# cvYouTian/Dedark-YOLO

Hardware: AMD Instinct MI355X
Metric: training img/s at 640x640 (higher is better)
Workload: dtype bf16

## Files before the change

dedark_yolo_amd/_C.py:

```python
import ctypes as C
import os

_HERE = os.path.dirname(os.path.abspath(__file__))
LIB_PATH = os.path.join(os.environ.get("DY_LIB_DIR") or os.path.join(_HERE, "lib"), "libdedark_yolo.so")

DY_F32, DY_BF16, DY_F16 = 0, 1, 2
ACT_NONE, ACT_SILU, ACT_LEAKY = 0, 1, 2
OPT_RULES = dict(Adam=0, Adamax=1, NAdam=2, RAdam=3, RMSProp=4)
STATS_REPLICAS = 64
BN_BWD_REPLICAS = 8

vp, i32, i64, f32, f64 = C.c_void_p, C.c_int, C.c_int64, C.c_float, C.c_double


class ConvDesc(C.Structure):
    _fields_ = [("src", vp), ("src_ld", i64), ("N", i32), ("Hs", i32), ("Ws", i32), ("Cs", i32), ("w", vp), ("dst", vp),
                ("dst_ld", i64), ("Hd", i32), ("Wd", i32), ("Cd", i32), ("KH", i32), ("KW", i32), ("stride", i32),
                ("pad", i32), ("dil", i32), ("scale", vp), ("shift", vp), ("act", i32), ("stats", vp), ("accumulate", i32),
                ("dtype", i32), ("dst_row_stride", i64), ("dst_img_stride", i64), ("KHf", i32), ("KWf", i32), ("kh0", i32),
                ("kh_step", i32), ("kw0", i32), ("kw_step", i32), ("dst_valid_channels", i32), ("dst_planar", vp),
                ("add_src", vp), ("add_src_ld", i64)]


class PackItem(C.Structure):
    _fields_ = [("w", vp), ("packed", vp), ("Cout", i32), ("Cout_pad", i32), ("Cin", i32), ("Cin_pad", i32), ("KH", i32),
                ("KW", i32), ("transposed", i32), ("dtype", i32), ("first_block", i64)]


class DetMaps(C.Structure):
    _fields_ = [("map", vp * 3), ("map_ld", i64 * 3), ("h", i32 * 3), ("w", i32 * 3), ("stride", f32 * 3), ("B", i32),
                ("nc", i32), ("n_levels", i32), ("dtype", i32)]


class DetMaps4(DetMaps):
    _fields_ = [("map3", vp), ("map_ld3", i64), ("h3", i32), ("w3", i32), ("stride3", f32)]


class AugSample(C.Structure):
    _fields_ = [("src", vp * 4), ("sh", i32 * 4), ("sw", i32 * 4), ("pitch", i64 * 4), ("rect", (i32 * 6) * 4), ("n_src", i32),
                ("canvas_h", i32), ("canvas_w", i32), ("hsv", i32), ("flipud", i32), ("fliplr", i32), ("minv", C.c_double * 6),
                ("lut", (C.c_uint8 * 256) * 3)]


class AugMixSample(C.Structure):
    _fields_ = [("a", AugSample), ("b", AugSample), ("r", C.c_double), ("r1", C.c_double), ("mix", i32)]


class SegDesc(C.Structure):
    _fields_ = [("mc", vp), ("mc_ld", i64), ("proto", vp), ("proto_ld", i64), ("B", i32), ("A", i32), ("nm", i32), ("mh", i32),
                ("mw", i32), ("target_gt_idx", vp), ("fg_mask", vp), ("target_box", vp), ("masks", vp), ("mask_dtype", i32),
                ("mask_h", i32), ("mask_w", i32), ("overlap", i32), ("gt_rows", vp), ("n_max", i32), ("img_h", f32), ("img_w", f32),
                ("pos", vp), ("npos", vp), ("dtype", i32)]


BIAS_GRAD_CHUNKS = 2048
LN_MAX_C = 2048
LN_MAX_PARTS = 512

POSE_MAX_LEVELS = 4
# ... 198 lines not shown
```

dedark_yolo_amd/csrc/conv.hip:

```cpp
#include <stdlib.h>
#include "dy_host.h"
#include "conv_epilogue.h"
#include "../../include/dedark_yolo.h"
#include "conv_route.h"

namespace {

constexpr int ROWB = 144;
constexpr int NTHREADS = 256;

struct ConvP {
  const char* src;
  long src_ld;
  int N, Hs, Ws, Cs;
  const char* w;
  char* dst;
  long dst_ld;
  int Hd, Wd, Cd;
  int KH, KW, stride, pad, dil;
  const float* scale;
  const float* shift;
  int act;
  double* stats;
  int accumulate;
// ... 629 lines not shown
  if (sl == 0 && co < Cout) {
    float t = 0.f;
#pragma unroll
    for (int u = 0; u < 8; ++u) t += red[u][cl];
    const int kh = tap / KW, kw = tap - kh * KW;
    g[(((long)co * Cin + ci) * KH + kh) * KW + kw] = t;
  }
}

template <typename T>
__global__ void pack_weight_kernel(const float* __restrict__ w, T* __restrict__ out, int Cout, int Cout_pad, int Cin,
                                   int Cin_pad, int KH, int KW, int transposed) {
  long total = (long)Cout_pad * KH * KW * Cin_pad;
  for (long i = blockIdx.x * (long)blockDim.x + threadIdx.x; i < total; i += (long)gridDim.x * blockDim.x) {
    int co, kh, kw, ci;
    long r = i;
    if (!transposed) {
      ci = (int)(r % Cin_pad); r /= Cin_pad;
      kw = (int)(r % KW); r /= KW;
      kh = (int)(r % KH); r /= KH;
      co = (int)r;
    } else {
      co = (int)(r % Cout_pad); r /= Cout_pad;
      kw = (int)(r % KW); r /= KW;
      kh = (int)(r % KH); r /= KH;
      ci = (int)r;
    }
    float v = (ci < Cin && co < Cout) ? w[(((long)co * Cin + ci) * KH + kh) * KW + kw] : 0.f;
    DT<T>::st(out + i, v);
  }
}

constexpr int PACK_TILE = 32, PACK_TAPS = 9;

__device__ inline void pack_store(const dy_pack_item& it, long o, float v) {
  if (it.dtype == DY_F32) ((float*)it.packed)[o] = v;
  else if (it.dtype == DY_F16) ((f16_t*)it.packed)[o] = (f16_t)v;
  else ((bf16_t*)it.packed)[o] = f32_to_bf16(v);
}

template <int TC>
__device__ inline void pack_chunk(const dy_pack_item& it, float (&tile)[PACK_TILE][PACK_TILE * PACK_TAPS + 1], int co0, int ci0, int T,
                                  int t0, int tc_rt) {
  const int tc = TC ? TC : tc_rt;
  const int tid = threadIdx.x;
  const int run = PACK_TILE * tc;
  {
    const int r = tid >> 3, co = co0 + r;
    const bool row_ok = co < it.Cout;
    const float* src = it.w + ((long)co * it.Cin + ci0) * T + t0;
    for (int k = tid & 7; k < run; k += 8) {
      const int cl = k / tc, t = k - cl * tc;
      const int ci = ci0 + cl;
      float v = 0.f;
      if (row_ok && ci < it.Cin) v = src[(long)cl * T + t];
      tile[r][cl * PACK_TAPS + t] = v;
    }
  }
  __syncthreads();
  const int VE = it.dtype == DY_F32 ? 4 : 8, GP = PACK_TILE / VE;
  const int n_vec = PACK_TILE * GP * tc;
  for (int i = tid; i < n_vec; i += 256) {
    const int g = i % GP, q = i / GP;
    const int a = q / tc, t = q - a * tc;
    float v[8];
    long o;
    bool ok;
    if (!it.transposed) {
      const int co = co0 + a, ci = ci0 + g * VE;
#pragma unroll
      for (int e = 0; e < 8; ++e) v[e] = e < VE ? tile[a][(g * VE + e) * PACK_TAPS + t] : 0.f;
      ok = co < it.Cout_pad && ci < it.Cin_pad;
      o = ((long)co * T + t0 + t) * it.Cin_pad + ci;
    } else {
      const int ci = ci0 + a, co = co0 + g * VE;
#pragma unroll
      for (int e = 0; e < 8; ++e) v[e] = e < VE ? tile[g * VE + e][a * PACK_TAPS + t] : 0.f;
      ok = co < it.Cout_pad && ci < it.Cin_pad;
      o = ((long)ci * T + t0 + t) * it.Cout_pad + co;
    }
    if (!ok) continue;
    if (it.dtype == DY_F32) stvec<float>((float*)it.packed + o, v);
    else if (it.dtype == DY_F16) stvec<f16_t>((f16_t*)it.packed + o, v);
    else stvec<bf16_t>((bf16_t*)it.packed + o, v);
  }
  __syncthreads();
}

__global__ __launch_bounds__(256) void pack_multi_kernel(const dy_pack_item* __restrict__ items, int n_items) {
  __shared__ float tile[PACK_TILE][PACK_TILE * PACK_TAPS + 1];
  __shared__ long fb[1024];
  const long b = blockIdx.x;
  const bool cached = n_items <= 1024;
  if (cached) {
    for (int i = threadIdx.x; i < n_items; i += 256) fb[i] = items[i].first_block;
    __syncthreads();
  }
  int lo = 0, hi = n_items - 1;
  while (lo < hi) {
    const int mid = (lo + hi + 1) >> 1;
    if ((cached ? fb[mid] : items[mid].first_block) <= b) lo = mid; else hi = mid - 1;
  }
  const dy_pack_item it = items[lo];
  const int tiles_ci = (it.Cin_pad + PACK_TILE - 1) / PACK_TILE;
  const int tb = (int)(b - it.first_block);
  const int co0 = (tb / tiles_ci) * PACK_TILE, ci0 = (tb % tiles_ci) * PACK_TILE;
  const int T = it.KH * it.KW;
  if (T == 9) pack_chunk<9>(it, tile, co0, ci0, 9, 0, 9);
  else if (T == 1) pack_chunk<1>(it, tile, co0, ci0, 1, 0, 1);
  else
    for (int t0 = 0; t0 < T; t0 += PACK_TAPS) pack_chunk<0>(it, tile, co0, ci0, T, t0, T - t0 < PACK_TAPS ? T - t0 : PACK_TAPS);
}

template <typename T, int MODE>
int launch_conv(const dy_conv_desc* d, hipStream_t st, const dy_conv_desc* classes, int ncls) {
  ConvP p;
  dy_route::fill_parity_classes(p, classes, ncls);
  dy_route::fill_gather(p, d);
  constexpr int BM = 128;
  const int tiles_m = dy_cdiv(p.M, BM);
  auto blocks = [&](int bn) {
    p.tiles_n = dy_cdiv(d->Cd, bn);
    p.nblk = tiles_m * p.tiles_n;
    if (p.ncls > 1) p.nblk = dy_route::number_parity_blocks(p, BM, dy_route::CLS_SEQUENTIAL);
  };
  dy_note_kernel(d->Cd <= 32 ? "conv_igemm_kernel<BN=32>" : (d->Cd <= 64 ? "conv_igemm_kernel<BN=64>" : "conv_igemm_kernel<BN=128>"));
  if (d->Cd <= 32) {
    blocks(32);
    conv_igemm_kernel<T, BM, 32, 4, 1, MODE><<<p.nblk, NTHREADS, 0, st>>>(p);
  } else if (d->Cd <= 64) {
    blocks(64);
    conv_igemm_kernel<T, BM, 64, 2, 2, MODE><<<p.nblk, NTHREADS, 0, st>>>(p);
  } else {
    blocks(128);
    conv_igemm_kernel<T, BM, 128, 2, 2, MODE><<<p.nblk, NTHREADS, 0, st>>>(p);
  }
  DY_LAUNCH_CHECK();
  return 0;
}

bool thin_eligible(const dy_conv_desc* d, int mode, bool parity_class = false) {
  static const bool off = dy_env("DY_NO_CONV_THIN") != nullptr;
  static const bool all_shapes = getenv("DY_CONV_THIN_ALL") != nullptr;
  if (off || d->dtype != DY_BF16) return false;
// ... 319 lines not shown
```

dedark_yolo_amd/csrc/optim.hip:

```cpp
#include "dy_host.h"
#include "../../include/dedark_yolo.h"

namespace {

struct Hyp { float lr[4]; float wd[4]; };

__global__ __launch_bounds__(256) void sumsq_kernel(const float* __restrict__ g, long n, double* acc) {
  __shared__ float sm[20];
  float s = 0.f;
  const long n4 = n >> 2;
  const f32x4* g4 = reinterpret_cast<const f32x4*>(g);
  for (long i = blockIdx.x * (long)blockDim.x + threadIdx.x; i < n4; i += (long)gridDim.x * blockDim.x) {
    f32x4 v = g4[i];
    s += v[0] * v[0] + v[1] * v[1] + v[2] * v[2] + v[3] * v[3];
  }
  if (blockIdx.x == 0 && threadIdx.x < (n & 3)) { float v = g[(n4 << 2) + threadIdx.x]; s += v * v; }
  s = block_sum(s, sm);
  if (threadIdx.x == 0) atomic_add_f64(acc, (double)s);
}

__device__ inline float step_coef(const double* sumsq, float max_norm, const float* loss_scale, bool* skip) {
  const float inv = loss_scale ? 1.f / loss_scale[0] : 1.f;
  *skip = false;
  if (!sumsq) return inv;
  const double ss = *sumsq;
  if (loss_scale && !(ss < (double)INFINITY)) {
    *skip = true;
    return 0.f;
  }
  const float nrm = (float)sqrt(ss) * inv;
  const float c = max_norm / (nrm + 1e-6f);
  return (c < 1.f ? c : 1.f) * inv;
}

__device__ inline float ema_mix(float e, float w, float ed) { return ed * e + (1.f - ed) * w; }

__global__ void sgd_kernel(float* __restrict__ p, const float* __restrict__ g, float* __restrict__ buf, float* __restrict__ ema,
                           const uint8_t* __restrict__ gid, Hyp h, float mom, int nesterov, float ed, const double* sumsq,
                           float max_norm, float gscale, const float* loss_scale, long n) {
  bool skip;
  const float cc = step_coef(sumsq, max_norm, loss_scale, &skip) * gscale;
  for (long i = blockIdx.x * (long)blockDim.x + threadIdx.x; i < n; i += (long)gridDim.x * blockDim.x) {
    if (skip) {
      if (ema) ema[i] = ema_mix(ema[i], p[i], ed);
      continue;
    }
    const int k = gid ? (gid[i] & 3) : 0;
    float w = p[i];
    float d = g[i] * cc + h.wd[k] * w;
    float b = mom * buf[i] + d;
    buf[i] = b;
// ... 150 lines not shown
    }
    if (ema) ema[i] = ema_mix(ema[i], w, ed);
  }
}

__global__ void loss_scale_update_kernel(float* st, const double* sumsq, float growth, float backoff, int interval) {
  if (threadIdx.x || blockIdx.x) return;
  if (!(*sumsq < (double)INFINITY)) {
    st[0] *= backoff;
    st[1] = 0.f;
    st[2] += 1.f;
  } else {
    const float good = st[1] + 1.f;
    if (good >= (float)interval) {
      st[0] *= growth;
      st[1] = 0.f;
    } else {
      st[1] = good;
    }
  }
}

__global__ void ema_lerp_kernel(float* __restrict__ ema, const float* __restrict__ src, float d, long n) {
  for (long i = blockIdx.x * (long)blockDim.x + threadIdx.x; i < n; i += (long)gridDim.x * blockDim.x)
    ema[i] = d * ema[i] + (1.f - d) * src[i];
}

constexpr int EW_CAP = 2048;

}

extern "C" int dy_sumsq(const float* g, int64_t n, double* acc, void* stream) {
  DY_CHECK(g && acc && n >= 0 && ((uintptr_t)g) % 16 == 0, "dy_sumsq: bad args");
  int blocks = dy_ew_blocks(n / 4 + 1, EW_CAP);
  if (blocks > 256) blocks = 256;
  sumsq_kernel<<<blocks, 256, 0, (hipStream_t)stream>>>(g, n, acc);
  DY_LAUNCH_CHECK();
  return 0;
}

extern "C" int dy_sgd_step_scaled(float* p, const float* g, float* mom_buf, float* ema, const uint8_t* group_id, float lr0, float lr1,
                                  float lr2, float wd0, float wd1, float wd2, float momentum, int nesterov, float ema_decay,
                                  const double* sumsq, float max_norm, float grad_scale, const float* loss_scale, int64_t n,
                                  void* stream) {
  DY_CHECK(p && g && mom_buf && n >= 0 && (!loss_scale || sumsq), "dy_sgd_step: bad args");
  if (n == 0) return 0;
  Hyp h = {{lr0, lr1, lr2, lr2}, {wd0, wd1, wd2, wd2}};
  sgd_kernel<<<dy_ew_blocks(n, EW_CAP), 256, 0, (hipStream_t)stream>>>(p, g, mom_buf, ema, group_id, h, momentum, nesterov, ema_decay, sumsq,
                                                            max_norm, grad_scale, loss_scale, n);
  DY_LAUNCH_CHECK();
  return 0;
}

extern "C" int dy_sgd_step(float* p, const float* g, float* mom_buf, float* ema, const uint8_t* group_id, float lr0, float lr1,
                           float lr2, float wd0, float wd1, float wd2, float momentum, int nesterov, float ema_decay,
                           const double* sumsq, float max_norm, float grad_scale, int64_t n, void* stream) {
  return dy_sgd_step_scaled(p, g, mom_buf, ema, group_id, lr0, lr1, lr2, wd0, wd1, wd2, momentum, nesterov, ema_decay, sumsq, max_norm,
                            grad_scale, nullptr, n, stream);
}

extern "C" int dy_adamw_step_scaled(float* p, const float* g, float* exp_avg, float* exp_avg_sq, float* ema, const uint8_t* group_id,
                                    float lr0, float lr1, float lr2, float wd0, float wd1, float wd2, float beta1, float beta2,
                                    float eps, int step, float ema_decay, const double* sumsq, float max_norm, float grad_scale,
                                    const float* loss_scale, int64_t n, void* stream) {
  DY_CHECK(p && g && exp_avg && exp_avg_sq && n >= 0 && step >= 1 && (!loss_scale || sumsq), "dy_adamw_step: bad args");
  if (n == 0) return 0;
  Hyp h = {{lr0, lr1, lr2, lr2}, {wd0, wd1, wd2, wd2}};
  adamw_kernel<<<dy_ew_blocks(n, EW_CAP), 256, 0, (hipStream_t)stream>>>(p, g, exp_avg, exp_avg_sq, ema, group_id, h, beta1, beta2, eps, step,
                                                              ema_decay, sumsq, max_norm, grad_scale, loss_scale, n);
// ... 73 lines not shown
```

dedark_yolo_amd/csrc/pool.hip:

```cpp
#include "dy_host.h"
#include "../../include/dedark_yolo.h"

namespace {

constexpr int EW_CAP = 4096;

template <typename T>
__global__ void maxpool_fwd_kernel(const T* __restrict__ x, long x_ld, T* __restrict__ y, long y_ld,
                                   uint8_t* __restrict__ arg, int N, int H, int W, int C, int k, int stride, int pad, int Ho,
                                   int Wo) {
  constexpr int VE = DT<T>::VE;
  const int CG = C / VE;
  const long total = (long)N * Ho * Wo * CG;
  for (long i = blockIdx.x * (long)blockDim.x + threadIdx.x; i < total; i += (long)gridDim.x * blockDim.x) {
    long px = i / CG;
    int c = (int)(i - px * CG) * VE;
    int wo = (int)(px % Wo);
    long t = px / Wo;
    int ho = (int)(t % Ho);
    int n = (int)(t / Ho);
    float best[VE];
    int bi[VE];
#pragma unroll
    for (int e = 0; e < VE; ++e) { best[e] = -INFINITY; bi[e] = 0; }
    bool first = true;
    for (int kh = 0; kh < k; ++kh) {
      int h = ho * stride - pad + kh;
      if (h < 0 || h >= H) continue;
      for (int kw = 0; kw < k; ++kw) {
        int w = wo * stride - pad + kw;
        if (w < 0 || w >= W) continue;
        float v[VE];
        ldvec<T>(x + (((long)n * H + h) * W + w) * x_ld + c, v);
#pragma unroll
        for (int e = 0; e < VE; ++e)
          if (first || v[e] > best[e] || v[e] != v[e]) { best[e] = v[e]; bi[e] = kh * k + kw; }
        first = false;
      }
    }
    stvec<T>(y + px * y_ld + c, best);
    if (arg) {
#pragma unroll
      for (int e = 0; e < VE; ++e) arg[px * C + c + e] = (uint8_t)bi[e];
    }
  }
}

template <typename T>
__global__ void maxpool_bwd_kernel(const T* __restrict__ dy, long dy_ld, const uint8_t* __restrict__ arg, T* __restrict__ dx,
                                   long dx_ld, int N, int H, int W, int C, int k, int stride, int pad, int Ho, int Wo,
                                   int accumulate) {
  constexpr int VE = DT<T>::VE;
  const int CG = C / VE;
  const long total = (long)N * H * W * CG;
  for (long i = blockIdx.x * (long)blockDim.x + threadIdx.x; i < total; i += (long)gridDim.x * blockDim.x) {
    long px = i / CG;
    int c = (int)(i - px * CG) * VE;
    int w = (int)(px % W);
    long t = px / W;
    int h = (int)(t % H);
    int n = (int)(t / H);
    float acc[VE];
#pragma unroll
    for (int e = 0; e < VE; ++e) acc[e] = 0.f;
    for (int kh = 0; kh < k; ++kh) {
      int th = h + pad - kh;
      if (th < 0 || th % stride) continue;
      int ho = th / stride;
      if (ho >= Ho) continue;
      for (int kw = 0; kw < k; ++kw) {
        int tw = w + pad - kw;
        if (tw < 0 || tw % stride) continue;
        int wo = tw / stride;
        if (wo >= Wo) continue;
        long opx = ((long)n * Ho + ho) * Wo + wo;
        float g[VE];
        ldvec<T>(dy + opx * dy_ld + c, g);
        const uint8_t* a = arg + opx * C + c;
#pragma unroll
        for (int e = 0; e < VE; ++e)
          if (a[e] == kh * k + kw) acc[e] += g[e];
      }
    }
    T* o = dx + px * dx_ld + c;
    if (accumulate) {
      float old[VE];
      ldvec<T>(o, old);
#pragma unroll
      for (int e = 0; e < VE; ++e) acc[e] += old[e];
    }
    stvec<T>(o, acc);
  }
}

template <typename T>
__global__ void upsample_fwd_kernel(const T* __restrict__ x, long x_ld, T* __restrict__ y, long y_ld, int N, int H, int W,
                                    int C, int s) {
  constexpr int VE = DT<T>::VE;
  const int CG = C / VE, Ho = H * s, Wo = W * s;
  const long total = (long)N * Ho * Wo * CG;
  for (long i = blockIdx.x * (long)blockDim.x + threadIdx.x; i < total; i += (long)gridDim.x * blockDim.x) {
    long px = i / CG;
    int c = (int)(i - px * CG) * VE;
    int wo = (int)(px % Wo);
    long t = px / Wo;
    int ho = (int)(t % Ho);
    int n = (int)(t / Ho);
    u32x4 v = *reinterpret_cast<const u32x4*>(x + (((long)n * H + ho / s) * W + wo / s) * x_ld + c);
    *reinterpret_cast<u32x4*>(y + px * y_ld + c) = v;
  }
}

template <typename T>
__global__ void upsample_bwd_kernel(const T* __restrict__ dy, long dy_ld, T* __restrict__ dx, long dx_ld, int N, int H, int W,
// ... 109 lines not shown
      if (x2) ldvec<T>(x2 + px * ld2 + g * VE, c);
      else { for (int e = 0; e < VE; ++e) c[e] = 0.f; }
#pragma unroll
      for (int e = 0; e < VE; ++e) { d0 += go[e] * a[e]; d1 += go[e] * b[e]; d2 += go[e] * c[e]; }
      T* p0 = dx0 + px * ldd0 + g * VE;
      T* p1 = dx1 + px * ldd1 + g * VE;
      T* p2 = dx2 + px * ldd2 + g * VE;
      if (acc0) ldvec<T>(p0, o); else { for (int e = 0; e < VE; ++e) o[e] = 0.f; }
#pragma unroll
      for (int e = 0; e < VE; ++e) o[e] += go[e] * w0;
      stvec<T>(p0, o);
      if (acc1) ldvec<T>(p1, o); else { for (int e = 0; e < VE; ++e) o[e] = 0.f; }
#pragma unroll
      for (int e = 0; e < VE; ++e) o[e] += go[e] * w1;
      stvec<T>(p1, o);
      if (x2) {
        if (acc2) ldvec<T>(p2, o); else { for (int e = 0; e < VE; ++e) o[e] = 0.f; }
#pragma unroll
        for (int e = 0; e < VE; ++e) o[e] += go[e] * w2;
        stvec<T>(p2, o);
      }
    }
    d0 = wave_sum(d0); d1 = wave_sum(d1); d2 = wave_sum(d2);
    if (lane == 0) {
      float dot = w0 * d0 + w1 * d1 + w2 * d2;
      DT<T>::st(dlg + px * lddl, w0 * (d0 - dot));
      DT<T>::st(dlg + px * lddl + 1, w1 * (d1 - dot));
      if (2 < lg_width) DT<T>::st(dlg + px * lddl + 2, w2 * (d2 - dot));
      for (int j = 3; j < lg_width; ++j) DT<T>::st(dlg + px * lddl + j, 0.f);
    }
  }
}

}

extern "C" int dy_maxpool_fwd(const void* x, int64_t x_ld, void* y, int64_t y_ld, uint8_t* argmax, int N, int H, int W, int C,
                              int k, int stride, int pad, int Ho, int Wo, int dtype, void* stream) {
  if (int e = dy_check_view("dy_maxpool_fwd(x)", x, x_ld, C, dtype)) return e;
  if (int e = dy_check_view("dy_maxpool_fwd(y)", y, y_ld, C, dtype)) return e;
  DY_CHECK(k >= 1 && k <= 15 && stride >= 1 && pad >= 0 && 2 * pad <= k, "dy_maxpool_fwd: bad window");
  DY_CHECK(Ho == (H + 2 * pad - k) / stride + 1 && Wo == (W + 2 * pad - k) / stride + 1, "dy_maxpool_fwd: bad output size");
  const int blocks = dy_ew_blocks((long)N * Ho * Wo * (C / dy_vec_elems(dtype)), EW_CAP);
  DY_DISPATCH_DTYPE("dy_maxpool_fwd", dtype,
                    maxpool_fwd_kernel<T><<<blocks, 256, 0, (hipStream_t)stream>>>((const T*)x, x_ld, (T*)y, y_ld, argmax, N, H, W, C, k,
                                                                                   stride, pad, Ho, Wo));
  DY_LAUNCH_CHECK();
  return 0;
}

extern "C" int dy_maxpool_bwd(const void* dy, int64_t dy_ld, const uint8_t* argmax, void* dx, int64_t dx_ld, int N, int H,
                              int W, int C, int k, int stride, int pad, int Ho, int Wo, int accumulate, int dtype,
                              void* stream) {
  if (int e = dy_check_view("dy_maxpool_bwd(dy)", dy, dy_ld, C, dtype)) return e;
  if (int e = dy_check_view("dy_maxpool_bwd(dx)", dx, dx_ld, C, dtype)) return e;
  DY_CHECK(argmax != nullptr, "dy_maxpool_bwd: null argmax");
  const int blocks = dy_ew_blocks((long)N * H * W * (C / dy_vec_elems(dtype)), EW_CAP);
  DY_DISPATCH_DTYPE("dy_maxpool_bwd", dtype,
                    maxpool_bwd_kernel<T><<<blocks, 256, 0, (hipStream_t)stream>>>((const T*)dy, dy_ld, argmax, (T*)dx, dx_ld, N, H, W, C,
                                                                                   k, stride, pad, Ho, Wo, accumulate));
  DY_LAUNCH_CHECK();
  return 0;
}

extern "C" int dy_upsample_nearest_fwd(const void* x, int64_t x_ld, void* y, int64_t y_ld, int N, int H, int W, int C, int scale,
                                       int dtype, void* stream) {
  if (int e = dy_check_view("dy_upsample_nearest_fwd(x)", x, x_ld, C, dtype)) return e;
  if (int e = dy_check_view("dy_upsample_nearest_fwd(y)", y, y_ld, C, dtype)) return e;
  DY_CHECK(scale >= 1, "dy_upsample_nearest_fwd: bad scale");
  const int blocks = dy_ew_blocks((long)N * H * scale * W * scale * (C / dy_vec_elems(dtype)), EW_CAP);
  DY_DISPATCH_DTYPE("dy_upsample_nearest_fwd", dtype,
                    upsample_fwd_kernel<T><<<blocks, 256, 0, (hipStream_t)stream>>>((const T*)x, x_ld, (T*)y, y_ld, N, H, W, C, scale));
  DY_LAUNCH_CHECK();
  return 0;
}

extern "C" int dy_upsample_nearest_bwd(const void* dy, int64_t dy_ld, void* dx, int64_t dx_ld, int N, int H, int W, int C,
                                       int scale, int accumulate, int dtype, void* stream) {
  if (int e = dy_check_view("dy_upsample_nearest_bwd(dy)", dy, dy_ld, C, dtype)) return e;
  if (int e = dy_check_view("dy_upsample_nearest_bwd(dx)", dx, dx_ld, C, dtype)) return e;
  const int blocks = dy_ew_blocks((long)N * H * W * (C / dy_vec_elems(dtype)), EW_CAP);
  DY_DISPATCH_DTYPE("dy_upsample_nearest_bwd", dtype,
                    upsample_bwd_kernel<T><<<blocks, 256, 0, (hipStream_t)stream>>>((const T*)dy, dy_ld, (T*)dx, dx_ld, N, H, W, C, scale,
                                                                                    accumulate));
  DY_LAUNCH_CHECK();
  return 0;
}

extern "C" int dy_copy2d(const void* src, int64_t src_ld, void* dst, int64_t dst_ld, int64_t pixels, int C, int accumulate,
                         int dtype, void* stream) {
  if (int e = dy_check_view("dy_copy2d(src)", src, src_ld, C, dtype)) return e;
  if (int e = dy_check_view("dy_copy2d(dst)", dst, dst_ld, C, dtype)) return e;
  const int blocks = dy_ew_blocks(pixels * (C / dy_vec_elems(dtype)), EW_CAP);
// ... 71 lines not shown
```

dedark_yolo_amd/ops.py:

```python
import ctypes as C
import math
import os
import weakref

import torch

from . import _C
from ._C import ACT_LEAKY, ACT_NONE, ACT_SILU, ConvDesc, DetMaps, DetMaps4, call

_compute_dtype = torch.float32
_pack_generation = 0
_weights_epoch = 0


def set_compute_dtype(dt):
    global _compute_dtype
    if dt not in (torch.float32, torch.bfloat16, torch.float16):
        raise ValueError(f"dedark_yolo_amd: unsupported compute dtype {dt}")
    _compute_dtype = dt


def get_compute_dtype():
    return _compute_dtype

# ... 191 lines not shown
    return w


def _pack(weight, cout_pad, cin_pad, transposed, dtype):
    key = (cout_pad, cin_pad, transposed, dtype)
    cache = weight.__dict__.setdefault("_dy_pack", {})
    hit = cache.get(key)
    tag = (_weights_epoch, weight._version)
    if hit is not None and hit[0] == tag:
        return hit[1]
    Co, Ci, KH, KW = weight.shape
    if hit is None:
        global _pack_generation
        _pack_generation += 1
    out = hit[1] if hit is not None else torch.empty(cout_pad * KH * KW * cin_pad, dtype=dtype, device=weight.device)
    w32 = _w32(weight)
    call("dy_pack_weight", ptr(w32), ptr(out), Co, cout_pad, Ci, cin_pad, KH, KW, 1 if transposed else 0, dt_id(dtype), stream())
    cache[key] = (tag, out)
    return out


_extra_pack_views = []


def register_pack_view(t):
    _extra_pack_views.append(weakref.ref(t))


class PackPlan:

    def __init__(self):
        self.sig = None
        self.table = None
        self.n_blocks = 0
        self._ent_key = None
        self._ent = []
        self._ent_sig = ()

    def _collect(self, model):
        ent = []
        _extra_pack_views[:] = [r for r in _extra_pack_views if r() is not None]
        for w in list(model.parameters()) + [r() for r in _extra_pack_views]:
            cache = w.__dict__.get("_dy_pack")
            if not cache or w.dtype != torch.float32 or not w.is_contiguous() or w.dim() != 4:
                continue
            for key, (tag, out) in cache.items():
                ent.append((w, key, out))
        return ent

    def repack(self, model):
        key = (id(model), _pack_generation)
        if key != self._ent_key:
            self._ent = self._collect(model)
            self._ent_sig = tuple((w.data_ptr(), out.data_ptr(), k) for w, k, out in self._ent)
            self._ent_key = key
        ent = self._ent
        if not ent:
            return
        sig = self._ent_sig
        if any(w.data_ptr() != sg[0] for (w, _, _), sg in zip(ent[:4], sig[:4])):
            self._ent_key = None
            return self.repack(model)
        if sig != self.sig:
            items = (_C.PackItem * len(ent))()
            blk = 0
            lib = _C.lib()
            for it, (w, (cout_pad, cin_pad, transposed, dtype), out) in zip(items, ent):
                Co, Ci, KH, KW = w.shape
                it.w, it.packed = w.data_ptr(), out.data_ptr()
                it.Cout, it.Cout_pad, it.Cin, it.Cin_pad, it.KH, it.KW = Co, cout_pad, Ci, cin_pad, KH, KW
                it.transposed, it.dtype, it.first_block = int(transposed), dt_id(dtype), blk
                blk += lib.dy_pack_item_blocks(cout_pad, cin_pad, KH, KW)
            raw = torch.frombuffer(bytearray(bytes(items)), dtype=torch.uint8)
            self.table = raw.to(ent[0][0].device)
            self.n_blocks, self.sig = blk, sig
        call("dy_pack_weights_multi", ptr(self.table), len(ent), self.n_blocks, stream())
        for w, key, out in ent:
            w.__dict__["_dy_pack"][key] = ((_weights_epoch, w._version), out)


def _padded_vec(v, n):
    if v is None:
        return None
    v = v.detach()
    if v.numel() == n and v.dtype == torch.float32:
        return v
    out = torch.zeros(n, dtype=torch.float32, device=v.device)
    out[:v.numel()] = v
    return out


def bn_fold(bn, cout_pad):
    tag = (_weights_epoch, bn.weight._version, bn.bias._version, bn.running_mean._version, bn.running_var._version,
           bn.weight.data_ptr(), bn.running_mean.data_ptr(), cout_pad)
    hit = bn.__dict__.get("_dy_fold")
    if hit is not None and hit[0] == tag:
        return hit[1]
    aff = hit[1] if (hit is not None and hit[1].shape[1] == cout_pad and hit[1].device == bn.weight.device) else \
        torch.empty((2, cout_pad), dtype=torch.float32, device=bn.weight.device)
    call("dy_bn_fold_eval_valid", ptr(bn.weight), ptr(bn.bias), ptr(bn.running_mean), ptr(bn.running_var), float(bn.eps),
         ptr(aff[0]), ptr(aff[1]), cout_pad, bn.weight.numel(), stream())
    bn.__dict__["_dy_fold"] = (tag, aff)
    return aff


def bn_fold_is_current(bn):
    hit = bn.__dict__.get("_dy_fold")
    return hit is not None and hit[0][:7] == (_weights_epoch, bn.weight._version, bn.bias._version, bn.running_mean._version,
                                               bn.running_var._version, bn.weight.data_ptr(), bn.running_mean.data_ptr())
# ... 1228 lines not shown
```

include/dedark_yolo.h:

```cpp
#ifndef DEDARK_YOLO_H
#define DEDARK_YOLO_H
#include <stddef.h>
#include <stdint.h>
#ifdef __cplusplus
extern "C" {
#endif

#define DY_F32 0
#define DY_BF16 1
#define DY_F16 2
#define DY_ACT_NONE 0
#define DY_ACT_SILU 1
#define DY_ACT_LEAKY 2
#define DY_STATS_REPLICAS 64
#define DY_BN_BWD_REPLICAS 8

const char* dy_last_error(void);
int dy_version(void);
const char* dy_last_kernel(void);
void dy_clear_last_kernel(void);

typedef struct {
  const void* src;
  int64_t src_ld;
// ... 2 lines not shown
  void* dst;
  int64_t dst_ld;
  int Hd, Wd, Cd;
  int KH, KW, stride, pad, dil;
  const float* scale;
  const float* shift;
  int act;
  double* stats;
  int accumulate;
  int dtype;
  int64_t dst_row_stride;
  int64_t dst_img_stride;
  int KHf, KWf;
  int kh0, kh_step;
  int kw0, kw_step;
  int dst_valid_channels;
  void* dst_planar;
  const void* add_src;
  int64_t add_src_ld;
} dy_conv_desc;

int dy_conv2d_fwd(const dy_conv_desc* d, void* stream);
int dy_conv2d_dgrad(const dy_conv_desc* d, void* stream);
int dy_conv2d_wgrad(const void* x, int64_t x_ld, int N, int Hi, int Wi, int Cin_pad, const void* dz, int64_t dz_ld, int Ho,
                    int Wo, int Cout_pad, int KH, int KW, int stride, int pad, int dil, int Cout, int Cin, float* scratch,
                    int64_t scratch_elems, float* g_oihw, int dtype, void* stream);
int dy_pack_weight(const float* w_oihw, void* packed, int Cout, int Cout_pad, int Cin, int Cin_pad, int KH, int KW,
                   int transposed, int dtype, void* stream);
typedef struct {
  const float* w;
  void* packed;
  int Cout, Cout_pad, Cin, Cin_pad, KH, KW, transposed, dtype;
  int64_t first_block;
} dy_pack_item;
int64_t dy_pack_item_blocks(int Cout_pad, int Cin_pad, int KH, int KW);
int dy_pack_weights_multi(const dy_pack_item* items_dev, int n_items, int64_t n_blocks, void* stream);

int dy_bn_finalize(const double* stats, int64_t count, const float* gamma, const float* beta, float* running_mean,
                   float* running_var, float momentum, float eps, float* scale, float* shift, float* mean, float* invstd,
                   int C, void* stream);
int dy_bn_fold_eval(const float* gamma, const float* beta, const float* running_mean, const float* running_var, float eps,
                    float* scale, float* shift, int C, void* stream);
int dy_bn_finalize_valid(const double* stats, int64_t count, const float* gamma, const float* beta, float* running_mean,
                         float* running_var, float momentum, float eps, float* scale, float* shift, float* mean, float* invstd,
                         int C, int C_valid, void* stream);
int dy_bn_fold_eval_valid(const float* gamma, const float* beta, const float* running_mean, const float* running_var, float eps,
                          float* scale, float* shift, int C, int C_valid, void* stream);
int dy_bn_act_fwd(const void* z, int64_t z_ld, const float* scale, const float* shift, int act, const void* residual,
                  int64_t res_ld, void* y, int64_t y_ld, int64_t pixels, int C, int dtype, void* stream);
int dy_bn_act_bwd_reduce(const void* dy, int64_t dy_ld, const void* z, int64_t z_ld, const float* scale,
                         const float* shift, const float* mean, const float* invstd, int act, int has_bn, double* sums,
                         int64_t pixels, int C, int dtype, void* stream);
int dy_bn_act_bwd_apply(const void* dy, int64_t dy_ld, const void* z, int64_t z_ld, const float* scale, const float* shift,
                        const float* mean, const float* invstd, const float* gamma, int act, int has_bn,
                        const double* sums, void* dz, int64_t dz_ld, float* dgamma, float* dbeta, int64_t pixels, int C,
                        int dtype, void* stream);
int dy_bn_act_bwd_apply_valid(const void* dy, int64_t dy_ld, const void* z, int64_t z_ld, const float* scale, const float* shift,
                              const float* mean, const float* invstd, const float* gamma, int act, int has_bn,
                              const double* sums, void* dz, int64_t dz_ld, float* dgamma, float* dbeta, int64_t pixels, int C,
                              int C_valid, int dtype, void* stream);

int dy_bn2_act_fwd(const void* u, int64_t u_ld, const void* v, int64_t v_ld, const float* scale_u, const float* shift_u,
                   const float* scale_v, const float* shift_v, int act, void* y, int64_t y_ld, int64_t pixels, int C, int dtype,
                   void* stream);
#define DY_BN2_MAX_PARTS 1024
int64_t dy_bn2_act_bwd_workspace(int64_t pixels, int C, int dtype);
// ... 300 lines not shown
```

Before: 1013.

## Merge plain/transposed weight packing, unroll sumsq, specialize maxpool windows

Weight packing now emits both the plain and transposed packed layouts from one read of the source tile. It stores converted 16-bit values in shared memory and finds its item with a wave-wide ballot search. The gradient sum-of-squares kernel uses eight independent accumulators with unrolled loads and a larger grid. Maxpool forward and backward are templated on common window shapes (5/1/2, 3/2/1, 2/2/0), with vectorized argmax byte loads and stores and a closed-form backward window. These target small per-step kernels (repacking, grad-norm, pooling), so the overall training gain is likely small, and the added index logic carries some correctness risk.

```diff
diff --git a/dedark_yolo_amd/_C.py b/dedark_yolo_amd/_C.py
--- a/dedark_yolo_amd/_C.py
+++ b/dedark_yolo_amd/_C.py
@@ -24,7 +24,7 @@
 
 class PackItem(C.Structure):
     _fields_ = [("w", vp), ("packed", vp), ("Cout", i32), ("Cout_pad", i32), ("Cin", i32), ("Cin_pad", i32), ("KH", i32),
-                ("KW", i32), ("transposed", i32), ("dtype", i32), ("first_block", i64)]
+                ("KW", i32), ("transposed", i32), ("dtype", i32), ("first_block", i64), ("packed_t", vp)]
 
 
 class DetMaps(C.Structure):
diff --git a/dedark_yolo_amd/csrc/conv.hip b/dedark_yolo_amd/csrc/conv.hip
--- a/dedark_yolo_amd/csrc/conv.hip
+++ b/dedark_yolo_amd/csrc/conv.hip
@@ -685,84 +685,123 @@
 }
 
 constexpr int PACK_TILE = 32, PACK_TAPS = 9;
-
-__device__ inline void pack_store(const dy_pack_item& it, long o, float v) {
-  if (it.dtype == DY_F32) ((float*)it.packed)[o] = v;
-  else if (it.dtype == DY_F16) ((f16_t*)it.packed)[o] = (f16_t)v;
-  else ((bf16_t*)it.packed)[o] = f32_to_bf16(v);
-}
-
-template <int TC>
-__device__ inline void pack_chunk(const dy_pack_item& it, float (&tile)[PACK_TILE][PACK_TILE * PACK_TAPS + 1], int co0, int ci0, int T,
-                                  int t0, int tc_rt) {
+constexpr int PACK_ROW_DW = PACK_TILE * PACK_TAPS / 2 + 1;
+
+__device__ inline int pack_find_item(const dy_pack_item* __restrict__ items, int n_items, long b) {
+  const int lane = threadIdx.x & 63;
+  int lo = 0, len = n_items;
+  while (len > 1) {
+    const int step = (len + 63) >> 6;
+    const int idx = lo + lane * step;
+    const bool le = idx < lo + len && items[idx].first_block <= b;
+    const int cnt = __popcll(__ballot(le));
+    const int nlo = lo + (cnt - 1) * step;
+    len = lo + len - nlo < step ? lo + len - nlo : step;
+    lo = nlo;
+  }
+  return __builtin_amdgcn_readfirstlane(lo);
+}
+
+template <typename E>
+__device__ inline E pack_cvt(float v, int dtype) {
+  if constexpr (sizeof(E) == 4) return v;
+  else return dtype == DY_F16 ? cvt16<f16_t>(v) : cvt16<bf16_t>(v);
+}
+
+template <typename E, int TC>
+__device__ inline void pack_chunk(const dy_pack_item& it, uint32_t* raw, int co0, int ci0, int T, int t0, int tc_rt) {
+  constexpr int VE = 16 / sizeof(E);
+  constexpr int CW = PACK_TILE * 2 / sizeof(E);
+  constexpr int RS = PACK_ROW_DW * 4 / sizeof(E);
+  E* tile = reinterpret_cast<E*>(raw);
   const int tc = TC ? TC : tc_rt;
   const int tid = threadIdx.x;
-  const int run = PACK_TILE * tc;
-  {
-    const int r = tid >> 3, co = co0 + r;
-    const bool row_ok = co < it.Cout;
-    const float* src = it.w + ((long)co * it.Cin + ci0) * T + t0;
-    for (int k = tid & 7; k < run; k += 8) {
-      const int cl = k / tc, t = k - cl * tc;
-      const int ci = ci0 + cl;
-      float v = 0.f;
-      if (row_ok && ci < it.Cin) v = src[(long)cl * T + t];
-      tile[r][cl * PACK_TAPS + t] = v;
+  const int run = CW * tc;
+  auto src_of = [&](int idx, int& r, int& k) -> const float* {
+    r = idx / run;
+    k = idx - r * run;
+    const int cl = k / tc, t = k - cl * tc;
+    const int co = co0 + r, ci = ci0 + cl;
+    k = cl * PACK_TAPS + t;
+    return (co < it.Cout && ci < it.Cin) ? it.w + ((long)co * it.Cin + ci) * T + t0 + t : nullptr;
+  };
+  if constexpr (TC != 0) {
+    constexpr int NL = PACK_TILE * CW * TC / 256;
+    float v[NL];
+#pragma unroll
+    for (int j = 0; j < NL; ++j) {
+      int r, k;
+      const float* p = src_of(tid + j * 256, r, k);
+      v[j] = p ? *p : 0.f;
+    }
+#pragma unroll
+    for (int j = 0; j < NL; ++j) {
+      int r, k;
+      src_of(tid + j * 256, r, k);
+      tile[r * RS + k] = pack_cvt<E>(v[j], it.dtype);
+    }
+  } else {
+    for (int idx = tid; idx < PACK_TILE * run; idx += 256) {
+      int r, k;
+      const float* p = src_of(idx, r, k);
+      tile[r * RS + k] = pack_cvt<E>(p ? *p : 0.f, it.dtype);
     }
   }
   __syncthreads();
-  const int VE = it.dtype == DY_F32 ? 4 : 8, GP = PACK_TILE / VE;
-  const int n_vec = PACK_TILE * GP * tc;
-  for (int i = tid; i < n_vec; i += 256) {
-    const int g = i % GP, q = i / GP;
-    const int a = q / tc, t = q - a * tc;
-    float v[8];
-    long o;
-    bool ok;
-    if (!it.transposed) {
+  E* plain = it.transposed ? nullptr : (E*)it.packed;
+  E* trans = it.transposed ? (E*)it.packed : (E*)it.packed_t;
+  typedef E vec_t __attribute__((ext_vector_type(VE)));
+  if (plain) {
+    constexpr int GP = CW / VE;
+    for (int i = tid; i < PACK_TILE * GP * tc; i += 256) {
+      const int g = i % GP, q = i / GP;
+      const int a = q / tc, t = q - a * tc;
       const int co = co0 + a, ci = ci0 + g * VE;
-#pragma unroll
-      for (int e = 0; e < 8; ++e) v[e] = e < VE ? tile[a][(g * VE + e) * PACK_TAPS + t] : 0.f;
-      ok = co < it.Cout_pad && ci < it.Cin_pad;
-      o = ((long)co * T + t0 + t) * it.Cin_pad + ci;
-    } else {
+      if (co >= it.Cout_pad || ci >= it.Cin_pad) continue;
+      vec_t v;
+#pragma unroll
+      for (int e = 0; e < VE; ++e) v[e] = tile[a * RS + (g * VE + e) * PACK_TAPS + t];
+      *reinterpret_cast<vec_t*>(plain + ((long)co * T + t0 + t) * it.Cin_pad + ci) = v;
+    }
+  }
+  if (trans) {
+    constexpr int GP = PACK_TILE / VE;
+    for (int i = tid; i < CW * GP * tc; i += 256) {
+      const int g = i % GP, q = i / GP;
+      const int a = q / tc, t = q - a * tc;
       const int ci = ci0 + a, co = co0 + g * VE;
-#pragma unroll
-      for (int e = 0; e < 8; ++e) v[e] = e < VE ? tile[g * VE + e][a * PACK_TAPS + t] : 0.f;
-      ok = co < it.Cout_pad && ci < it.Cin_pad;
-      o = ((long)ci * T + t0 + t) * it.Cout_pad + co;
-    }
-    if (!ok) continue;
-    if (it.dtype == DY_F32) stvec<float>((float*)it.packed + o, v);
-    else if (it.dtype == DY_F16) stvec<f16_t>((f16_t*)it.packed + o, v);
-    else stvec<bf16_t>((bf16_t*)it.packed + o, v);
+      if (co >= it.Cout_pad || ci >= it.Cin_pad) continue;
+      vec_t v;
+#pragma unroll
+      for (int e = 0; e < VE; ++e) v[e] = tile[(g * VE + e) * RS + a * PACK_TAPS + t];
+      *reinterpret_cast<vec_t*>(trans + ((long)ci * T + t0 + t) * it.Cout_pad + co) = v;
+    }
   }
   __syncthreads();
 }
 
+template <typename E>
+__device__ inline void pack_tile(const dy_pack_item& it, uint32_t* raw, int co0, int ci0) {
+  const int T = it.KH * it.KW;
+  if (T == 9) pack_chunk<E, 9>(it, raw, co0, ci0, 9, 0, 9);
+  else if (T == 1) pack_chunk<E, 1>(it, raw, co0, ci0, 1, 0, 1);
+  else
+    for (int t0 = 0; t0 < T; t0 += PACK_TAPS) pack_chunk<E, 0>(it, raw, co0, ci0, T, t0, T - t0 < PACK_TAPS ? T - t0 : PACK_TAPS);
+}
+
 __global__ __launch_bounds__(256) void pack_multi_kernel(const dy_pack_item* __restrict__ items, int n_items) {
-  __shared__ float tile[PACK_TILE][PACK_TILE * PACK_TAPS + 1];
-  __shared__ long fb[1024];
+  __shared__ uint32_t raw[PACK_TILE * PACK_ROW_DW];
   const long b = blockIdx.x;
-  const bool cached = n_items <= 1024;
-  if (cached) {
-    for (int i = threadIdx.x; i < n_items; i += 256) fb[i] = items[i].first_block;
-    __syncthreads();
-  }
-  int lo = 0, hi = n_items - 1;
-  while (lo < hi) {
-    const int mid = (lo + hi + 1) >> 1;
-    if ((cached ? fb[mid] : items[mid].first_block) <= b) lo = mid; else hi = mid - 1;
-  }
-  const dy_pack_item it = items[lo];
+  const dy_pack_item it = items[pack_find_item(items, n_items, b)];
   const int tiles_ci = (it.Cin_pad + PACK_TILE - 1) / PACK_TILE;
   const int tb = (int)(b - it.first_block);
   const int co0 = (tb / tiles_ci) * PACK_TILE, ci0 = (tb % tiles_ci) * PACK_TILE;
-  const int T = it.KH * it.KW;
-  if (T == 9) pack_chunk<9>(it, tile, co0, ci0, 9, 0, 9);
-  else if (T == 1) pack_chunk<1>(it, tile, co0, ci0, 1, 0, 1);
-  else
-    for (int t0 = 0; t0 < T; t0 += PACK_TAPS) pack_chunk<0>(it, tile, co0, ci0, T, t0, T - t0 < PACK_TAPS ? T - t0 : PACK_TAPS);
+  if (it.dtype == DY_F32) {
+    pack_tile<float>(it, raw, co0, ci0);
+    if (ci0 + PACK_TILE / 2 < it.Cin_pad) pack_tile<float>(it, raw, co0, ci0 + PACK_TILE / 2);
+  } else {
+    pack_tile<uint16_t>(it, raw, co0, ci0);
+  }
 }
 
 template <typename T, int MODE>
diff --git a/dedark_yolo_amd/csrc/optim.hip b/dedark_yolo_amd/csrc/optim.hip
--- a/dedark_yolo_amd/csrc/optim.hip
+++ b/dedark_yolo_amd/csrc/optim.hip
@@ -5,18 +5,37 @@
 
 struct Hyp { float lr[4]; float wd[4]; };
 
+constexpr int SUMSQ_UNROLL = 8;
+
 __global__ __launch_bounds__(256) void sumsq_kernel(const float* __restrict__ g, long n, double* acc) {
   __shared__ float sm[20];
-  float s = 0.f;
+  float s[SUMSQ_UNROLL];
+#pragma unroll
+  for (int u = 0; u < SUMSQ_UNROLL; ++u) s[u] = 0.f;
   const long n4 = n >> 2;
   const f32x4* g4 = reinterpret_cast<const f32x4*>(g);
-  for (long i = blockIdx.x * (long)blockDim.x + threadIdx.x; i < n4; i += (long)gridDim.x * blockDim.x) {
-    f32x4 v = g4[i];
-    s += v[0] * v[0] + v[1] * v[1] + v[2] * v[2] + v[3] * v[3];
-  }
-  if (blockIdx.x == 0 && threadIdx.x < (n & 3)) { float v = g[(n4 << 2) + threadIdx.x]; s += v * v; }
-  s = block_sum(s, sm);
-  if (threadIdx.x == 0) atomic_add_f64(acc, (double)s);
+  constexpr long CHUNK = SUMSQ_UNROLL * 256;
+  for (long base = blockIdx.x * CHUNK; base < n4; base += (long)gridDim.x * CHUNK) {
+    const long i0 = base + threadIdx.x;
+    if (base + CHUNK <= n4) {
+      f32x4 v[SUMSQ_UNROLL];
+#pragma unroll
+      for (int u = 0; u < SUMSQ_UNROLL; ++u) v[u] = g4[i0 + u * 256];
+#pragma unroll
+      for (int u = 0; u < SUMSQ_UNROLL; ++u) s[u] += v[u][0] * v[u][0] + v[u][1] * v[u][1] + v[u][2] * v[u][2] + v[u][3] * v[u][3];
+    } else {
+#pragma unroll
+      for (int u = 0; u < SUMSQ_UNROLL; ++u)
+        if (i0 + u * 256 < n4) {
+          const f32x4 v = g4[i0 + u * 256];
+          s[u] += v[0] * v[0] + v[1] * v[1] + v[2] * v[2] + v[3] * v[3];
+        }
+    }
+  }
+  if (blockIdx.x == 0 && threadIdx.x < (n & 3)) { float v = g[(n4 << 2) + threadIdx.x]; s[0] += v * v; }
+  float t = ((s[0] + s[1]) + (s[2] + s[3])) + ((s[4] + s[5]) + (s[6] + s[7]));
+  t = block_sum(t, sm);
+  if (threadIdx.x == 0) atomic_add_f64(acc, (double)t);
 }
 
 __device__ inline float step_coef(const double* sumsq, float max_norm, const float* loss_scale, bool* skip) {
@@ -233,9 +252,9 @@
 
 extern "C" int dy_sumsq(const float* g, int64_t n, double* acc, void* stream) {
   DY_CHECK(g && acc && n >= 0 && ((uintptr_t)g) % 16 == 0, "dy_sumsq: bad args");
-  int blocks = dy_ew_blocks(n / 4 + 1, EW_CAP);
-  if (blocks > 256) blocks = 256;
-  sumsq_kernel<<<blocks, 256, 0, (hipStream_t)stream>>>(g, n, acc);
+  long blocks = (n / 4 + SUMSQ_UNROLL * 256) / (SUMSQ_UNROLL * 256);
+  if (blocks > 512) blocks = 512;
+  sumsq_kernel<<<(unsigned)blocks, 256, 0, (hipStream_t)stream>>>(g, n, acc);
   DY_LAUNCH_CHECK();
   return 0;
 }
diff --git a/dedark_yolo_amd/csrc/pool.hip b/dedark_yolo_amd/csrc/pool.hip
--- a/dedark_yolo_amd/csrc/pool.hip
+++ b/dedark_yolo_amd/csrc/pool.hip
@@ -5,11 +5,37 @@
 
 constexpr int EW_CAP = 4096;
 
-template <typename T>
-__global__ void maxpool_fwd_kernel(const T* __restrict__ x, long x_ld, T* __restrict__ y, long y_ld,
-                                   uint8_t* __restrict__ arg, int N, int H, int W, int C, int k, int stride, int pad, int Ho,
-                                   int Wo) {
-  constexpr int VE = DT<T>::VE;
+constexpr int POOL_CAP = 16384;
+
+template <int VE>
+__device__ inline uint64_t ld_arg(const uint8_t* a, bool vec) {
+  if (vec) {
+    if constexpr (VE == 8) return *reinterpret_cast<const uint64_t*>(a);
+    else return *reinterpret_cast<const uint32_t*>(a);
+  }
+  uint64_t r = 0;
+#pragma unroll
+  for (int e = 0; e < VE; ++e) r |= (uint64_t)a[e] << (8 * e);
+  return r;
+}
+template <int VE>
+__device__ inline void st_arg(uint8_t* a, uint64_t bits, bool vec) {
+  if (vec) {
+    if constexpr (VE == 8) *reinterpret_cast<uint64_t*>(a) = bits;
+    else *reinterpret_cast<uint32_t*>(a) = (uint32_t)bits;
+    return;
+  }
+#pragma unroll
+  for (int e = 0; e < VE; ++e) a[e] = (uint8_t)(bits >> (8 * e));
+}
+
+template <typename T, int K, int S, int P>
+__global__ __launch_bounds__(256) void maxpool_fwd_kernel(const T* __restrict__ x, long x_ld, T* __restrict__ y, long y_ld,
+                                                          uint8_t* __restrict__ arg, int N, int H, int W, int C, int k_rt,
+                                                          int stride_rt, int pad_rt, int Ho, int Wo, int arg_vec) {
+  constexpr int VE = DT<T>::VE;
+  constexpr int UN = K ? K : 1;
+  const int k = K ? K : k_rt, stride = K ? S : stride_rt, pad = K ? P : pad_rt;
   const int CG = C / VE;
   const long total = (long)N * Ho * Wo * CG;
   for (long i = blockIdx.x * (long)blockDim.x + threadIdx.x; i < total; i += (long)gridDim.x * blockDim.x) {
@@ -19,19 +45,24 @@
     long t = px / Wo;
     int ho = (int)(t % Ho);
     int n = (int)(t / Ho);
+    const int h0 = ho * stride - pad, w0 = wo * stride - pad;
+    const T* xn = x + (long)n * H * W * x_ld + c;
     float best[VE];
     int bi[VE];
 #pragma unroll
     for (int e = 0; e < VE; ++e) { best[e] = -INFINITY; bi[e] = 0; }
     bool first = true;
+#pragma unroll UN
     for (int kh = 0; kh < k; ++kh) {
-      int h = ho * stride - pad + kh;
+      const int h = h0 + kh;
       if (h < 0 || h >= H) continue;
+      const T* xr = xn + (long)h * W * x_ld;
+#pragma unroll UN
       for (int kw = 0; kw < k; ++kw) {
-        int w = wo * stride - pad + kw;
+        const int w = w0 + kw;
         if (w < 0 || w >= W) continue;
         float v[VE];
-        ldvec<T>(x + (((long)n * H + h) * W + w) * x_ld + c, v);
+        ldvec<T>(xr + (long)w * x_ld, v);
 #pragma unroll
         for (int e = 0; e < VE; ++e)
           if (first || v[e] > best[e] || v[e] != v[e]) { best[e] = v[e]; bi[e] = kh * k + kw; }
@@ -40,17 +71,22 @@
     }
     stvec<T>(y + px * y_ld + c, best);
     if (arg) {
-#pragma unroll
-      for (int e = 0; e < VE; ++e) arg[px * C + c + e] = (uint8_t)bi[e];
-    }
-  }
-}
-
-template <typename T>
-__global__ void maxpool_bwd_kernel(const T* __restrict__ dy, long dy_ld, const uint8_t* __restrict__ arg, T* __restrict__ dx,
-                                   long dx_ld, int N, int H, int W, int C, int k, int stride, int pad, int Ho, int Wo,
-                                   int accumulate) {
-  constexpr int VE = DT<T>::VE;
+      uint64_t bits = 0;
+#pragma unroll
+      for (int e = 0; e < VE; ++e) bits |= (uint64_t)(uint8_t)bi[e] << (8 * e);
+      st_arg<VE>(arg + px * C + c, bits, arg_vec);
+    }
+  }
+}
+
+template <typename T, int K, int S, int P>
+__global__ __launch_bounds__(256) void maxpool_bwd_kernel(const T* __restrict__ dy, long dy_ld, const uint8_t* __restrict__ arg,
+                                                          T* __restrict__ dx, long dx_ld, int N, int H, int W, int C, int k_rt,
+                                                          int stride_rt, int pad_rt, int Ho, int Wo, int accumulate, int arg_vec) {
+  constexpr int VE = DT<T>::VE;
+  constexpr int UN = K ? (K + S - 1) / S : 1;
+  const int k = K ? K : k_rt, stride = K ? S : stride_rt, pad = K ? P : pad_rt;
+  const int nwin = (k + stride - 1) / stride;
   const int CG = C / VE;
   const long total = (long)N * H * W * CG;
   for (long i = blockIdx.x * (long)blockDim.x + threadIdx.x; i < total; i += (long)gridDim.x * blockDim.x) {
@@ -60,26 +96,28 @@
     long t = px / W;
     int h = (int)(t % H);
     int n = (int)(t / H);
+    const int ho_top = (h + pad) / stride, wo_top = (w + pad) / stride;
+    const long on = (long)n * Ho * Wo;
     float acc[VE];
 #pragma unroll
     for (int e = 0; e < VE; ++e) acc[e] = 0.f;
-    for (int kh = 0; kh < k; ++kh) {
-      int th = h + pad - kh;
-      if (th < 0 || th % stride) continue;
-      int ho = th / stride;
-      if (ho >= Ho) continue;
-      for (int kw = 0; kw < k; ++kw) {
-        int tw = w + pad - kw;
-        if (tw < 0 || tw % stride) continue;
-        int wo = tw / stride;
-        if (wo >= Wo) continue;
-        long opx = ((long)n * Ho + ho) * Wo + wo;
+#pragma unroll UN
+    for (int jh = 0; jh < nwin; ++jh) {
+      const int ho = ho_top - jh, kh = h + pad - ho * stride;
+      const bool h_ok = kh < k && ho >= 0 && ho < Ho;
+      const long orow = on + (long)(ho < 0 ? 0 : (ho >= Ho ? Ho - 1 : ho)) * Wo;
+#pragma unroll UN
+      for (int jw = 0; jw < nwin; ++jw) {
+        const int wo = wo_top - jw, kw = w + pad - wo * stride;
+        const bool ok = h_ok && kw < k && wo >= 0 && wo < Wo;
+        const long opx = orow + (wo < 0 ? 0 : (wo >= Wo ? Wo - 1 : wo));
         float g[VE];
         ldvec<T>(dy + opx * dy_ld + c, g);
-        const uint8_t* a = arg + opx * C + c;
+        const uint64_t a = ld_arg<VE>(arg + opx * C + c, arg_vec);
+        const int tap = ok ? kh * k + kw : 256;
 #pragma unroll
         for (int e = 0; e < VE; ++e)
-          if (a[e] == kh * k + kw) acc[e] += g[e];
+          if ((int)((a >> (8 * e)) & 0xff) == tap) acc[e] += g[e];
       }
     }
     T* o = dx + px * dx_ld + c;
@@ -255,6 +293,8 @@
   }
 }
 
+inline bool pool_window(int k, int s, int p, int K, int S, int P) { return k == K && s == S && p == P; }
+
 }
 
 extern "C" int dy_maxpool_fwd(const void* x, int64_t x_ld, void* y, int64_t y_ld, uint8_t* argmax, int N, int H, int W, int C,
@@ -263,10 +303,17 @@
   if (int e = dy_check_view("dy_maxpool_fwd(y)", y, y_ld, C, dtype)) return e;
   DY_CHECK(k >= 1 && k <= 15 && stride >= 1 && pad >= 0 && 2 * pad <= k, "dy_maxpool_fwd: bad window");
   DY_CHECK(Ho == (H + 2 * pad - k) / stride + 1 && Wo == (W + 2 * pad - k) / stride + 1, "dy_maxpool_fwd: bad output size");
-  const int blocks = dy_ew_blocks((long)N * Ho * Wo * (C / dy_vec_elems(dtype)), EW_CAP);
-  DY_DISPATCH_DTYPE("dy_maxpool_fwd", dtype,
-                    maxpool_fwd_kernel<T><<<blocks, 256, 0, (hipStream_t)stream>>>((const T*)x, x_ld, (T*)y, y_ld, argmax, N, H, W, C, k,
-                                                                                   stride, pad, Ho, Wo));
+  const int ve = dy_vec_elems(dtype);
+  const int blocks = dy_ew_blocks((long)N * Ho * Wo * (C / ve), POOL_CAP);
+  const int arg_vec = ((uintptr_t)argmax) % ve == 0;
+  hipStream_t st = (hipStream_t)stream;
+  DY_DISPATCH_DTYPE("dy_maxpool_fwd", dtype, {
+    auto kernel = pool_window(k, stride, pad, 5, 1, 2)   ? maxpool_fwd_kernel<T, 5, 1, 2>
+                  : pool_window(k, stride, pad, 3, 2, 1) ? maxpool_fwd_kernel<T, 3, 2, 1>
+                  : pool_window(k, stride, pad, 2, 2, 0) ? maxpool_fwd_kernel<T, 2, 2, 0>
+                                                         : maxpool_fwd_kernel<T, 0, 0, 0>;
+    kernel<<<blocks, 256, 0, st>>>((const T*)x, x_ld, (T*)y, y_ld, argmax, N, H, W, C, k, stride, pad, Ho, Wo, arg_vec);
+  });
   DY_LAUNCH_CHECK();
   return 0;
 }
@@ -277,10 +324,19 @@
   if (int e = dy_check_view("dy_maxpool_bwd(dy)", dy, dy_ld, C, dtype)) return e;
   if (int e = dy_check_view("dy_maxpool_bwd(dx)", dx, dx_ld, C, dtype)) return e;
   DY_CHECK(argmax != nullptr, "dy_maxpool_bwd: null argmax");
-  const int blocks = dy_ew_blocks((long)N * H * W * (C / dy_vec_elems(dtype)), EW_CAP);
-  DY_DISPATCH_DTYPE("dy_maxpool_bwd", dtype,
-                    maxpool_bwd_kernel<T><<<blocks, 256, 0, (hipStream_t)stream>>>((const T*)dy, dy_ld, argmax, (T*)dx, dx_ld, N, H, W, C,
-                                                                                   k, stride, pad, Ho, Wo, accumulate));
+  DY_CHECK(k >= 1 && k <= 15 && stride >= 1 && pad >= 0 && 2 * pad <= k, "dy_maxpool_bwd: bad window");
+  DY_CHECK(Ho == (H + 2 * pad - k) / stride + 1 && Wo == (W + 2 * pad - k) / stride + 1, "dy_maxpool_bwd: bad output size");
+  const int ve = dy_vec_elems(dtype);
+  const int blocks = dy_ew_blocks((long)N * H * W * (C / ve), POOL_CAP);
+  const int arg_vec = ((uintptr_t)argmax) % ve == 0;
+  hipStream_t st = (hipStream_t)stream;
+  DY_DISPATCH_DTYPE("dy_maxpool_bwd", dtype, {
+    auto kernel = pool_window(k, stride, pad, 5, 1, 2)   ? maxpool_bwd_kernel<T, 5, 1, 2>
+                  : pool_window(k, stride, pad, 3, 2, 1) ? maxpool_bwd_kernel<T, 3, 2, 1>
+                  : pool_window(k, stride, pad, 2, 2, 0) ? maxpool_bwd_kernel<T, 2, 2, 0>
+                                                         : maxpool_bwd_kernel<T, 0, 0, 0>;
+    kernel<<<blocks, 256, 0, st>>>((const T*)dy, dy_ld, argmax, (T*)dx, dx_ld, N, H, W, C, k, stride, pad, Ho, Wo, accumulate, arg_vec);
+  });
   DY_LAUNCH_CHECK();
   return 0;
 }
diff --git a/dedark_yolo_amd/ops.py b/dedark_yolo_amd/ops.py
--- a/dedark_yolo_amd/ops.py
+++ b/dedark_yolo_amd/ops.py
@@ -247,6 +247,7 @@
     def __init__(self):
         self.sig = None
         self.table = None
+        self.n_items = 0
         self.n_blocks = 0
         self._ent_key = None
         self._ent = []
@@ -277,19 +278,27 @@
             self._ent_key = None
             return self.repack(model)
         if sig != self.sig:
-            items = (_C.PackItem * len(ent))()
+            merged = {}
+            for w, (cout_pad, cin_pad, transposed, dtype), out in ent:
+                pair = merged.setdefault((id(w), cout_pad, cin_pad, dtype), [w, None, None])
+                pair[2 if transposed else 1] = out
+            items = (_C.PackItem * len(merged))()
             blk = 0
             lib = _C.lib()
-            for it, (w, (cout_pad, cin_pad, transposed, dtype), out) in zip(items, ent):
+            for it, ((_, cout_pad, cin_pad, dtype), (w, plain, trans)) in zip(items, merged.items()):
                 Co, Ci, KH, KW = w.shape
-                it.w, it.packed = w.data_ptr(), out.data_ptr()
+                it.w = w.data_ptr()
                 it.Cout, it.Cout_pad, it.Cin, it.Cin_pad, it.KH, it.KW = Co, cout_pad, Ci, cin_pad, KH, KW
-                it.transposed, it.dtype, it.first_block = int(transposed), dt_id(dtype), blk
+                if plain is not None:
+                    it.packed, it.transposed, it.packed_t = plain.data_ptr(), 0, None if trans is None else trans.data_ptr()
+                else:
+                    it.packed, it.transposed, it.packed_t = trans.data_ptr(), 1, None
+                it.dtype, it.first_block = dt_id(dtype), blk
                 blk += lib.dy_pack_item_blocks(cout_pad, cin_pad, KH, KW)
             raw = torch.frombuffer(bytearray(bytes(items)), dtype=torch.uint8)
             self.table = raw.to(ent[0][0].device)
-            self.n_blocks, self.sig = blk, sig
-        call("dy_pack_weights_multi", ptr(self.table), len(ent), self.n_blocks, stream())
+            self.n_items, self.n_blocks, self.sig = len(merged), blk, sig
+        call("dy_pack_weights_multi", ptr(self.table), self.n_items, self.n_blocks, stream())
         for w, key, out in ent:
             w.__dict__["_dy_pack"][key] = ((_weights_epoch, w._version), out)
 
diff --git a/include/dedark_yolo.h b/include/dedark_yolo.h
--- a/include/dedark_yolo.h
+++ b/include/dedark_yolo.h
@@ -58,6 +58,7 @@
   void* packed;
   int Cout, Cout_pad, Cin, Cin_pad, KH, KW, transposed, dtype;
   int64_t first_block;
+  void* packed_t;
 } dy_pack_item;
 int64_t dy_pack_item_blocks(int Cout_pad, int Cin_pad, int KH, int KW);
 int dy_pack_weights_multi(const dy_pack_item* items_dev, int n_items, int64_t n_blocks, void* stream);
```

Result: no change. 1017, median of 6 (+0.5%).
